# Safari77/rupphash

Measured on AMD Instinct MI355X. Metric: pdq_hashes_per_sec_512x512_rgb, higher is better.
Workload: dtype f32

## Files before the change

rupphash_amd/csrc/pdq_fused512.hip:

```cpp
#include "pdq_tail.hpp"
#include "rph_internal.h"

namespace {

typedef _Float16 h2 __attribute__((ext_vector_type(2)));
typedef _Float16 h8 __attribute__((ext_vector_type(8)));

template <int SW_, int CH_ = 3, bool PARK_ = true>
struct Geo {
    static constexpr int SW = SW_;
    static constexpr int CH = CH_;
    static constexpr int NSTRIP = 512 / SW;
    static constexpr int CL = SW / 8;
    static constexpr int NG = 64 / CL;
    static constexpr int NH = 64 / (NG * 8);
    static constexpr int NOCT = SW / 8;
    static constexpr int TILE_PITCH = SW * 2 + 16;
    static constexpr int TILE_BYTES = 64 * TILE_PITCH;
    static constexpr int OFF_TILE = 0;
    static constexpr int OFF_XCHG = NH == 2 ? 32 * TILE_PITCH : 0;
    static constexpr int OFF_STATE = TILE_BYTES;
    static constexpr int OFF_EDGE = OFF_STATE + 7168;
#ifndef RPH_PARK_CHAINS
#define RPH_PARK_CHAINS 1
#endif
    static constexpr bool PARK = RPH_PARK_CHAINS && PARK_ && SW == 64;
    static constexpr int OFF_PARK_C = OFF_EDGE + 1536;
    static constexpr int OFF_PARK_E = OFF_PARK_C + (PARK ? 9 * 64 * 4 : 0);
    static constexpr int LDS_BYTES = OFF_PARK_E + (PARK ? 9 * 6 * 4 : 0);
    static constexpr int WAVES_PER_SIMD = 2;
    static_assert(64 * 33 * 4 <= TILE_BYTES, "sample transpose buffer must fit in the dead V tile");
    static_assert((NG - 1) * 7 * CL * 16 <= (NH == 2 ? 32 : 64) * TILE_PITCH, "exchange area must fit");
    static_assert(rph::TAIL_LDS_FLOATS * 4 <= TILE_BYTES, "tail scratch must fit in the dead V tile");
};
constexpr int SAMP_PITCH = 33;

struct Px8 {
    uint32_t d[6];
};
struct __attribute__((packed, aligned(4))) U3 {
    uint32_t x, y, z;
};

struct __attribute__((packed, aligned(4))) U2 {
    uint32_t x, y;
};
template <int CH = 3>
__device__ __forceinline__ Px8 load_px8(const uint8_t *p)
{
    Px8 r;
    if (CH == 1) {
        const U2 a = *reinterpret_cast<const U2 *>(p);
        r.d[0] = a.x; r.d[1] = a.y; r.d[2] = r.d[3] = r.d[4] = r.d[5] = 0;
        return r;
    }
    const U3 a = *reinterpret_cast<const U3 *>(p);
    const U3 b = *reinterpret_cast<const U3 *>(p + 12);
    r.d[0] = a.x; r.d[1] = a.y; r.d[2] = a.z; r.d[3] = b.x; r.d[4] = b.y; r.d[5] = b.z;
    return r;
}

template <int P>
__device__ __forceinline__ float luma_px(const Px8 &v)
{
    constexpr int B = 3 * P;
    const float r = (float)((v.d[B >> 2] >> (8 * (B & 3))) & 0xFFu);
    const float g = (float)((v.d[(B + 1) >> 2] >> (8 * ((B + 1) & 3))) & 0xFFu);
    const float b = (float)((v.d[(B + 2) >> 2] >> (8 * ((B + 2) & 3))) & 0xFFu);
    const float num = __builtin_fmaf(299.0f, r, __builtin_fmaf(587.0f, g, __builtin_fmaf(114.0f, b, 500.0f)));
    return __builtin_truncf(num * 0.001f);
}

template <int CH = 3>
__device__ __forceinline__ void luma8(const Px8 &v, float (&l)[8])
{
    if (CH == 1) {
#pragma unroll
        for (int i = 0; i < 8; i++) l[i] = (float)((v.d[i >> 2] >> (8 * (i & 3))) & 0xFFu);
        return;
    }
    l[0] = luma_px<0>(v); l[1] = luma_px<1>(v); l[2] = luma_px<2>(v); l[3] = luma_px<3>(v);
    l[4] = luma_px<4>(v); l[5] = luma_px<5>(v); l[6] = luma_px<6>(v); l[7] = luma_px<7>(v);
}

constexpr uint32_t BIASED_ZERO = 0x64006400u;
struct Row8 {
    h2 q[4];
};
__device__ __forceinline__ h2 h2_bits(uint32_t u) { return __builtin_bit_cast(h2, u); }
__device__ __forceinline__ h2 byte_pair_lo(uint32_t d) { return h2_bits(__builtin_amdgcn_perm(0x64646464u, d, 0x04010400u)); }
__device__ __forceinline__ h2 byte_pair_hi(uint32_t d) { return h2_bits(__builtin_amdgcn_perm(0x64646464u, d, 0x04030402u)); }

__device__ __forceinline__ float dot2_from_zero(h2 a, h2 k, uint32_t after)
{
    float r;
    asm volatile("v_dot2_f32_f16 %0, %1, %2, 0" : "=v"(r) : "v"(__builtin_bit_cast(uint32_t, a)), "s"(__builtin_bit_cast(uint32_t, k)), "v"(after));
    return r;
}

struct Pairs12 {
    h2 P[12];
};
__device__ __forceinline__ Pairs12 byte_pairs(const Px8 &v)
{
    Pairs12 r;
#pragma unroll
    for (int i = 0; i < 6; i++) {
        r.P[2 * i] = byte_pair_lo(v.d[i]);
        r.P[2 * i + 1] = byte_pair_hi(v.d[i]);
    }
    return r;
}
__device__ __forceinline__ Row8 luma_row(const Pairs12 &pr, bool zero, uint32_t &order)
{
    const h2 *P = pr.P;
    const h2 k_rg = h2{(_Float16)299.0f, (_Float16)587.0f};
    const h2 k_b0 = h2{(_Float16)114.0f, (_Float16)0.0f};
    const h2 k_0r = h2{(_Float16)0.0f, (_Float16)299.0f};
    const h2 k_gb = h2{(_Float16)587.0f, (_Float16)114.0f};
    float vhalf;
    asm("v_mov_b32 %0, 0.5" : "=v"(vhalf));
    h2 packed[4];
#pragma unroll
    for (int pp = 0; pp < 4; pp++) {
        const float n0 = __builtin_amdgcn_fdot2(P[3 * pp], k_rg, dot2_from_zero(P[3 * pp + 1], k_b0, order), false);
        const float n1 = __builtin_amdgcn_fdot2(P[3 * pp + 1], k_0r, dot2_from_zero(P[3 * pp + 2], k_gb, order), false);
        const float y0 = __builtin_fmaf(n0, 0.001f, vhalf), y1 = __builtin_fmaf(n1, 0.001f, vhalf);
        packed[pp] = __builtin_bit_cast(h2, __builtin_amdgcn_cvt_pkrtz(y0, y1));
    }
    order = __builtin_bit_cast(uint32_t, packed[3]);
    Row8 r;
#pragma unroll
    for (int i = 0; i < 4; i++) {
        r.q[i] = packed[i];
        if (zero) r.q[i] = h2_bits(BIASED_ZERO);
    }
    return r;
}
__device__ __forceinline__ Row8 luma_row_gray(const Px8 &v, bool zero, uint32_t &order)
{
    Row8 r;
    r.q[0] = byte_pair_lo(v.d[0]);
    r.q[1] = byte_pair_hi(v.d[0]);
    r.q[2] = byte_pair_lo(v.d[1]);
    r.q[3] = byte_pair_hi(v.d[1]);
#pragma unroll
    for (int i = 0; i < 4; i++)
        if (zero) r.q[i] = h2_bits(BIASED_ZERO);
    order = __builtin_bit_cast(uint32_t, r.q[3]);
    return r;
}
template <int CH = 3>
__device__ __forceinline__ Row8 pack_row(const Px8 &v, bool zero, uint32_t &order)
{
    if (CH == 1) return luma_row_gray(v, zero, order);
    return luma_row(byte_pairs(v), zero, order);
}
__device__ __forceinline__ uint4 row_bits(const Row8 &r)
{
    uint4 u;
    u.x = __builtin_bit_cast(uint32_t, r.q[0]);
    u.y = __builtin_bit_cast(uint32_t, r.q[1]);
    u.z = __builtin_bit_cast(uint32_t, r.q[2]);
    u.w = __builtin_bit_cast(uint32_t, r.q[3]);
    return u;
}
__device__ __forceinline__ Row8 bits_row(const uint4 &u)
{
    Row8 r;
    r.q[0] = __builtin_bit_cast(h2, u.x);
    r.q[1] = __builtin_bit_cast(h2, u.y);
    r.q[2] = __builtin_bit_cast(h2, u.z);
    r.q[3] = __builtin_bit_cast(h2, u.w);
    return r;
}

__device__ __forceinline__ float div_small(float N, float d, float dinv)
{
    const float q0 = N * dinv;
    const float r = __builtin_fmaf(-q0, d, N);
    return __builtin_fmaf(r, dinv, q0);
}

__device__ __forceinline__ void wave_lds_fence() { asm volatile("" ::: "memory"); }

struct Wave {
    uint8_t *lds;
    const uint8_t *img;
    size_t row_stride;
    uint32_t rs32;
    int lane;
    float hs, sum, ring[8];
    uint4 pv;
    float row_d8, row_dinv8;
    float smp[32];
    float smp_last;
    float csum, cring[8];
    float ecs, ering[8];
    float bnew[8];
    rph::TailAcc tail;
    bool want_quality;
};

template <class G>
__device__ __forceinline__ int half_row(int b, int h, int g, int k) { return 64 * b + 4 + (G::NG * 8) * h + 8 * g + k; }

template <class G>
__device__ __forceinline__ void half_offsets(const Wave &w, int b, int s, int h, uint32_t &off0, uint32_t &off_max)
{
    const int c = w.lane & (G::CL - 1), g = w.lane / G::CL;
    const uint32_t col = (uint32_t)(G::SW * s + 8 * c) * (uint32_t)G::CH;
    off0 = (uint32_t)half_row<G>(b, h, g, 0) * w.rs32 + col;
    off_max = 511u * w.rs32 + col;
}
template <int CH>
__device__ __forceinline__ Px8 load_px8_at(const Wave &w, uint32_t off) { return load_px8<CH>(w.img + off); }

template <class G>
__device__ __forceinline__ void half_issue(const Wave &w, int b, int s, int h, Px8 (&pre)[8])
{
    uint32_t off, off_max;
    half_offsets<G>(w, b, s, h, off, off_max);
#pragma unroll
    for (int k = 0; k < 8; k++) {
        pre[k] = load_px8_at<G::CH>(w, off);
        off = off + w.rs32;
        off = off < off_max ? off : off_max;
    }
}

template <class G, bool LAST_BAND>
__device__ __forceinline__ void half_luma(const Wave &w, int b, int h, Px8 (&pre)[8], Row8 (&L)[8], bool has_next, int nb, int ns, int nh)
{
    const int g = w.lane / G::CL;
    uint32_t off, off_max;
    half_offsets<G>(w, nb, ns, nh, off, off_max);
    uint32_t order = 0;
#pragma unroll
    for (int k = 0; k < 8; k++) {
        if (G::CH == 1) {
            const Px8 cur = pre[k];
            if (has_next) pre[k] = load_px8_at<1>(w, off);
            off = off + w.rs32;
            off = off < off_max ? off : off_max;
            L[k] = luma_row_gray(cur, LAST_BAND && (half_row<G>(b, h, g, k) >= 512), order);
            continue;
        }
        const Pairs12 pr = byte_pairs(pre[k]);
        if (has_next) pre[k] = load_px8_at<3>(w, off);
        off = off + w.rs32;
        off = off < off_max ? off : off_max;
        L[k] = luma_row(pr, LAST_BAND && (half_row<G>(b, h, g, k) >= 512), order);
    }
}

template <class G>
__device__ __forceinline__ void half_build(Wave &w, int s, int h, const Row8 (&L)[8])
{
    const int c = w.lane & (G::CL - 1), g = w.lane / G::CL;
    uint8_t *tile = w.lds + G::OFF_TILE;
    uint8_t *xchg = w.lds + G::OFF_XCHG;
    uint8_t *state = w.lds + G::OFF_STATE + (G::SW * s + 8 * c) * 2;

    if (g < G::NG - 1) {
        uint8_t *x = xchg + ((g * 7) * G::CL + c) * 16;
#pragma unroll
        for (int k = 1; k < 8; k++) *reinterpret_cast<uint4 *>(x + (k - 1) * (G::CL * 16)) = row_bits(L[k]);
    }
    wave_lds_fence();
    Row8 hist[7];
    {
        const uint8_t *hp = (g == 0) ? state : xchg + (((g - 1) * 7) * G::CL + c) * 16;
        const int stride = (g == 0) ? 1024 : G::CL * 16;
#pragma unroll
        for (int j = 0; j < 7; j++) hist[j] = bits_row(*reinterpret_cast<const uint4 *>(hp + j * stride));
    }
    wave_lds_fence();
    if (g == G::NG - 1) {
#pragma unroll
        for (int k = 1; k < 8; k++) *reinterpret_cast<uint4 *>(state + (k - 1) * 1024) = row_bits(L[k]);
    }
    const int row0 = (G::NG * 8) * h + 8 * g;
    Row8 v;
#pragma unroll
    for (int i = 0; i < 4; i++) {
        const h2 two_bias = h2{(_Float16)2048.0f, (_Float16)2048.0f};
        h2 a = hist[0].q[i] + (hist[1].q[i] - two_bias);
        h2 bb = hist[2].q[i] + (hist[3].q[i] - two_bias);
        h2 cc = hist[4].q[i] + (hist[5].q[i] - two_bias);
        h2 dd = hist[6].q[i] + (L[0].q[i] - two_bias);
        v.q[i] = (a + bb) + (cc + dd);
    }
    *reinterpret_cast<uint4 *>(tile + (row0 + 0) * G::TILE_PITCH + 16 * c) = row_bits(v);
#pragma unroll
    for (int m = 1; m < 8; m++) {
#pragma unroll
        for (int i = 0; i < 4; i++) v.q[i] = (v.q[i] - hist[m - 1].q[i]) + L[m].q[i];
        *reinterpret_cast<uint4 *>(tile + (row0 + m) * G::TILE_PITCH + 16 * c) = row_bits(v);
    }
    wave_lds_fence();
}

__device__ __forceinline__ uint32_t h2_diff(uint32_t cur, uint32_t prev)
{
    return __builtin_bit_cast(uint32_t, __builtin_bit_cast(h2, cur) - __builtin_bit_cast(h2, prev));
}
template <int HI>
__device__ __forceinline__ float hs_step(float hs, uint32_t packed)
{
    float r;
    if (HI)
        asm("v_fma_mix_f32 %0, %1, 1.0, %2 op_sel:[1,0,0] op_sel_hi:[1,0,0]" : "=v"(r) : "v"(packed), "v"(hs));
    else
        asm("v_fma_mix_f32 %0, %1, 1.0, %2 op_sel:[0,0,0] op_sel_hi:[1,0,0]" : "=v"(r) : "v"(packed), "v"(hs));
    return r;
}
template <int HI>
__device__ __forceinline__ float hs_sub(float hs, uint32_t packed)
{
    float r;
    if (HI)
        asm("v_fma_mix_f32 %0, %1, -1.0, %2 op_sel:[1,0,0] op_sel_hi:[1,0,0]" : "=v"(r) : "v"(packed), "v"(hs));
    else
        asm("v_fma_mix_f32 %0, %1, -1.0, %2 op_sel:[0,0,0] op_sel_hi:[1,0,0]" : "=v"(r) : "v"(packed), "v"(hs));
    return r;
}

template <int E>
__device__ __forceinline__ void row_step(Wave &w, float in2)
{
    constexpr int slot = (E + 4) & 7;
    w.sum = w.sum + in2;
    w.sum = w.sum - w.ring[slot];
    w.ring[slot] = in2;
}

template <bool EDGE_ROWS>
__device__ __forceinline__ float pass1_value(const Wave &w, float hs)
{
    if (EDGE_ROWS) return div_small(hs, w.row_d8, w.row_dinv8);
    return hs;
}

template <class G, bool EDGE_ROWS, bool FIRST, bool LAST>
__device__ __forceinline__ void scan_strip(Wave &w)
{
    const int r = w.lane;
    const uint8_t *tp = w.lds + G::OFF_TILE + r * G::TILE_PITCH;
    const float *edge = reinterpret_cast<const float *>(w.lds + G::OFF_EDGE);
    float fresh[G::NOCT];
#pragma unroll
    for (int q = 0; q < G::NOCT; q++) {
        const uint4 cur = *reinterpret_cast<const uint4 *>(tp + 16 * q);
        const uint32_t dq[4] = {h2_diff(cur.x, w.pv.x), h2_diff(cur.y, w.pv.y), h2_diff(cur.z, w.pv.z), h2_diff(cur.w, w.pv.w)};
        const bool first_octet = FIRST && q == 0;
        float e0 = 0.f, e1 = 0.f, e2 = 0.f;
        if (first_octet) {
            e0 = edge[0 * 64 + r];
            e1 = edge[1 * 64 + r];
            e2 = edge[2 * 64 + r];
        }
#define RPH_STEP(E)                                                              \
    {                                                                            \
        w.hs = hs_step<(E) & 1>(w.hs, dq[(E) >> 1]);                             \
        float in2 = pass1_value<EDGE_ROWS>(w, w.hs);                             \
        if (first_octet && (E) == 4) in2 = e0;                                   \
        if (first_octet && (E) == 5) in2 = e1;                                   \
        if (first_octet && (E) == 6) in2 = e2;                                   \
        if (!(first_octet && (E) < 4)) row_step<E>(w, in2);  \
    }
        RPH_STEP(0) RPH_STEP(1) RPH_STEP(2) RPH_STEP(3) RPH_STEP(4)
        fresh[q] = w.sum * 0.125f;
        RPH_STEP(5) RPH_STEP(6) RPH_STEP(7)
#undef RPH_STEP
        w.pv = cur;
    }
    if (LAST) {
        const float e3 = edge[3 * 64 + r], e4 = edge[4 * 64 + r], e5 = edge[5 * 64 + r];
        w.hs = hs_sub<0>(w.hs, w.pv.x); row_step<0>(w, e3);
        w.hs = hs_sub<1>(w.hs, w.pv.x); row_step<1>(w, e4);
        w.hs = hs_sub<0>(w.hs, w.pv.y); row_step<2>(w, e5);
        w.hs = hs_sub<1>(w.hs, w.pv.y);
        {
            const float in511 = (EDGE_ROWS ? div_small(w.hs, w.row_d8, w.row_dinv8) : w.hs) * 2.0f;
            row_step<3>(w, in511);
        }
        w.sum = w.sum - w.ring[0];
        w.smp_last = w.sum / 7.0f;
    }
#pragma unroll
    for (int i = 0; i < 32 - G::NOCT; i++) w.smp[i] = w.smp[i + G::NOCT];
#pragma unroll
    for (int q = 0; q < G::NOCT; q++) w.smp[32 - G::NOCT + q] = fresh[q];
}

__device__ __forceinline__ void scan_reset(Wave &w, int b)
{
    w.hs = 0.f;
    w.sum = 0.f;
#pragma unroll
    for (int i = 0; i < 8; i++) w.ring[i] = 0.f;
    w.pv = make_uint4(0, 0, 0, 0);
    const int y = 64 * b + w.lane;
    const int lo = y - 3 < 0 ? 0 : y - 3, hi = y + 4 > 511 ? 511 : y + 4;
    const float d = (float)(hi - lo + 1);
    w.row_d8 = d * 0.125f;
    w.row_dinv8 = (1.0f / d) * 8.0f;
}

template <class G>
__device__ __forceinline__ void col_pass(Wave &w, int b, bool second_half)
{
    float *tb = reinterpret_cast<float *>(w.lds + G::OFF_TILE);
#pragma unroll
    for (int t = 0; t < 32; t++) tb[w.lane * SAMP_PITCH + t] = w.smp[t];
    tb[w.lane * SAMP_PITCH + 32] = w.smp_last;
    wave_lds_fence();
    const bool active = second_half ? (w.lane >= 31) : (w.lane < 31);
    if (active) {
        float *park = reinterpret_cast<float *>(w.lds + G::OFF_PARK_C) + w.lane;
        if (G::PARK) {
            w.csum = park[0];
#pragma unroll
            for (int e = 0; e < 8; e++) w.cring[e] = park[64 * (e + 1)];
        }
        const float *samp = tb + (second_half ? w.lane - 31 : w.lane + 1);
#pragma unroll
        for (int u = 0; u < 8; u++) {
            float in[8];
#pragma unroll
            for (int e = 0; e < 8; e++) in[e] = samp[(8 * u + e) * SAMP_PITCH];
#pragma unroll
            for (int e = 0; e < 8; e++) {
                w.csum = w.csum + in[e];
                w.csum = w.csum - w.cring[e];
                w.cring[e] = in[e];
                if (e == 0) w.bnew[u] = w.csum * (0.125f * 0.015625f);
            }
        }
        if (G::PARK) {
            park[0] = w.csum;
#pragma unroll
            for (int e = 0; e < 8; e++) park[64 * (e + 1)] = w.cring[e];
        }
    }
    wave_lds_fence();
}

template <int CH>
__device__ __forceinline__ void edge_rowvals(const Wave &w, int y, bool live, float (&rv)[6])
{
    const int yc = y > 511 ? 511 : y;
    const Px8 pl = load_px8<CH>(w.img + (size_t)yc * w.row_stride);
    const Px8 pr = load_px8<CH>(w.img + (size_t)yc * w.row_stride + 504 * CH);
    float l[8], r[8];
    luma8<CH>(pl, l);
    luma8<CH>(pr, r);
    const float r0 = (((l[0] + l[1]) + l[2]) + l[3]) + l[4];
    const float r1 = r0 + l[5];
    const float r2 = r1 + l[6];
    const float q510 = (((r[3] + r[4]) + r[5]) + r[6]) + r[7];
    const float q509 = q510 + r[2];
    const float q508 = q509 + r[1];
    rv[0] = div_small(r0 * 64.0f, 5.0f, 1.0f / 5.0f);
    rv[1] = div_small(r1 * 64.0f, 6.0f, 1.0f / 6.0f);
    rv[2] = div_small(r2 * 64.0f, 7.0f, 1.0f / 7.0f);
    rv[3] = div_small(q508 * 64.0f, 7.0f, 1.0f / 7.0f);
    rv[4] = div_small(q509 * 64.0f, 6.0f, 1.0f / 6.0f);
    rv[5] = div_small(q510 * 64.0f, 5.0f, 1.0f / 5.0f);
    if (!live) {
#pragma unroll
        for (int k = 0; k < 6; k++) rv[k] = 0.f;
    }
}

template <class G>
__device__ __forceinline__ void edge_prologue(Wave &w)
{
    float *edge = reinterpret_cast<float *>(w.lds + G::OFF_EDGE);
    float rv[6];
    edge_rowvals<G::CH>(w, w.lane & 3, true, rv);
    if (w.lane < 4) {
#pragma unroll
        for (int k = 0; k < 6; k++) edge[k * 64 + w.lane] = rv[k];
    }
    wave_lds_fence();
    w.ecs = 0.f;
#pragma unroll
    for (int i = 0; i < 8; i++) w.ering[i] = 0.f;
    if (w.lane < 6) {
#pragma unroll
        for (int t = 0; t < 4; t++) {
            const float v = edge[w.lane * 64 + t];
            w.ecs = w.ecs + v;
            w.ering[t] = v;
        }
        if (G::PARK) {
            float *park = reinterpret_cast<float *>(w.lds + G::OFF_PARK_E) + w.lane;
            park[0] = w.ecs;
#pragma unroll
            for (int i = 0; i < 8; i++) park[6 * (i + 1)] = w.ering[i];
        }
    }
    wave_lds_fence();
}

template <class G, int KIND>
__device__ __forceinline__ void edge_band(Wave &w, int b)
{
    float *edge = reinterpret_cast<float *>(w.lds + G::OFF_EDGE);
    {
        float rv[6];
        const int y = 64 * b + 4 + w.lane;
        edge_rowvals<G::CH>(w, y, y < 512, rv);
#pragma unroll
        for (int k = 0; k < 6; k++) edge[k * 64 + w.lane] = rv[k];
    }
    wave_lds_fence();
    if (w.lane < 6) {
        float *mine = edge + w.lane * 64;
        float *park = reinterpret_cast<float *>(w.lds + G::OFF_PARK_E) + w.lane;
        if (G::PARK) {
            w.ecs = park[0];
#pragma unroll
            for (int i = 0; i < 8; i++) w.ering[i] = park[6 * (i + 1)];
        }
#pragma unroll 1
        for (int u = 0; u < 8; u++) {
            float in[8], out[8];
#pragma unroll
            for (int e = 0; e < 8; e++) in[e] = mine[8 * u + e];
#pragma unroll
            for (int e = 0; e < 8; e++) {
                constexpr int dummy = 0;
                (void)dummy;
                const int slot = (e + 4) & 7;
                const bool add = !(KIND == 2 && u == 7 && e >= 4);
                if (add) w.ecs = w.ecs + in[e];
                w.ecs = w.ecs - w.ering[slot];
                w.ering[slot] = in[e];
                float o;
                if (KIND == 0 && u == 0 && e < 3)
                    o = w.ecs / (float)(5 + e);
                else if (KIND == 2 && u == 7 && e >= 4)
                    o = w.ecs / (float)(11 - e);
                else
                    o = w.ecs * 0.125f;
                out[e] = o;
            }
#pragma unroll
            for (int e = 0; e < 8; e++) mine[8 * u + e] = out[e];
        }
        if (G::PARK) {
            park[0] = w.ecs;
#pragma unroll
            for (int i = 0; i < 8; i++) park[6 * (i + 1)] = w.ering[i];
        }
    }
    wave_lds_fence();
}

template <class G>
__device__ __forceinline__ void store_samples(const Wave &w, float *band_samples, bool second_half)
{
    float *p = band_samples + (second_half ? 32 * 64 : 0) + w.lane;
    asm volatile("" : "+v"(p));
#pragma unroll
    for (int t = 0; t < 32; t++) p[t * 64] = w.smp[t];
    if (second_half) p[32 * 64] = w.smp_last;
}

template <class G, int KIND, bool LL = false>
__device__ __forceinline__ void do_band(Wave &w, int b, Px8 (&pre)[8], float *samples = nullptr)
{
    constexpr bool EDGE_ROWS = KIND != 1;
    if (!LL) edge_band<G, KIND>(w, b);
    scan_reset(w, b);
#pragma unroll 1
    for (int s = 0; s < G::NSTRIP; s++) {
#pragma unroll 1
        for (int h = 0; h < G::NH; h++) {
            Row8 L[8];
            int nb = b, ns = s, nh = h + 1;
            if (nh == G::NH) {
                nh = 0;
                ns = s + 1;
                if (ns == G::NSTRIP) {
                    ns = 0;
                    nb = b + 1;
                }
            }
            half_luma<G, KIND == 2>(w, b, h, pre, L, LL ? nb == b : nb < 8, nb, ns, nh);
            half_build<G>(w, s, h, L);
        }
        if (s == 0)
            scan_strip<G, EDGE_ROWS, true, false>(w);
        else if (s == G::NSTRIP - 1)
            scan_strip<G, EDGE_ROWS, false, true>(w);
        else
            scan_strip<G, EDGE_ROWS, false, false>(w);
        wave_lds_fence();
        if (LL) {
            if (s == G::NSTRIP / 2 - 1) store_samples<G>(w, samples, false);
            if (s == G::NSTRIP - 1) store_samples<G>(w, samples, true);
        } else {
            if (s == G::NSTRIP / 2 - 1) col_pass<G>(w, b, false);
            if (s == G::NSTRIP - 1) col_pass<G>(w, b, true);
        }
        wave_lds_fence();
    }
    if (LL) return;
#pragma unroll
    for (int u = 0; u < 8; u++)
        if (KIND != 0 || u > 0) rph::tail_row(w.tail, w.bnew[u], 8 * b + u - 1, w.lane, w.want_quality);
}

template <class G>
__global__ void __launch_bounds__(64, G::WAVES_PER_SIMD) pdq_fused512_kernel(const uint8_t *__restrict__ px, uint32_t n, size_t row_stride,
                                                          size_t image_stride, uint8_t *hash, float *quality, float *coeffs,
                                                          uint8_t *dihedral, uint8_t *valid)
{
    __shared__ __attribute__((aligned(16))) uint8_t lds[G::LDS_BYTES];
    const uint32_t img = blockIdx.x;
    Wave w;
    w.lds = lds;
    w.img = px + (size_t)img * image_stride;
    w.row_stride = row_stride;
    w.rs32 = (uint32_t)row_stride;
    w.lane = threadIdx.x;
    w.csum = 0.f;
    w.smp_last = 0.f;
#pragma unroll
    for (int i = 0; i < 32; i++) w.smp[i] = 0.f;
#pragma unroll
    for (int i = 0; i < 8; i++) w.cring[i] = 0.f;
    if (G::PARK) {
#pragma unroll
        for (int i = 0; i < 9; i++) reinterpret_cast<float *>(lds + G::OFF_PARK_C)[64 * i + w.lane] = 0.f;
    }
    rph::tail_init(w.tail);
    w.want_quality = quality != nullptr;
#pragma unroll
    for (int u = 0; u < 8; u++) w.bnew[u] = 0.f;

    {
        for (int j = 0; j < 3; j++)
            for (int t = w.lane; t < 64; t += 64) *reinterpret_cast<uint4 *>(lds + G::OFF_STATE + j * 1024 + t * 16) = make_uint4(BIASED_ZERO, BIASED_ZERO, BIASED_ZERO, BIASED_ZERO);
        uint32_t order = 0;
#pragma unroll 1
        for (int it = 0; it < 4; it++) {
            const int slot = it * 64 + w.lane;
            const int chunk = slot & 63, row = slot >> 6;
            const Px8 p = load_px8<G::CH>(w.img + (size_t)row * row_stride + (size_t)(8 * chunk) * G::CH);
            *reinterpret_cast<uint4 *>(lds + G::OFF_STATE + (3 + row) * 1024 + (8 * chunk) * 2) = row_bits(pack_row<G::CH>(p, false, order));
        }
    }
    edge_prologue<G>(w);

    Px8 pre[8];
    half_issue<G>(w, 0, 0, 0, pre);
    do_band<G, 0>(w, 0, pre);
#pragma unroll 1
    for (int b = 1; b < 7; b++) do_band<G, 1>(w, b, pre);
    do_band<G, 2>(w, 7, pre);

    if (G::PARK) {
        w.csum = reinterpret_cast<const float *>(lds + G::OFF_PARK_C)[w.lane];
        w.cring[0] = reinterpret_cast<const float *>(lds + G::OFF_PARK_C)[64 + w.lane];
    }
    w.csum = w.csum - w.cring[0];
    rph::tail_row(w.tail, (w.csum / 7.0f) * 0.015625f, 63, w.lane, w.want_quality);

    __syncthreads();
    rph::tail_finish(w.tail, reinterpret_cast<float *>(lds), w.lane, hash + (size_t)img * 32, quality ? quality + img : nullptr,
                  coeffs ? coeffs + (size_t)img * 256 : nullptr, dihedral ? dihedral + (size_t)img * 256 : nullptr);
    if (valid && w.lane == 0) valid[img] = 1;
}

constexpr int LL_SAMPLE_FLOATS = 8 * 65 * 64;
constexpr int LL_EDGE_PITCH = 520;

template <class G, int KIND>
__device__ __forceinline__ void ll_band(Wave &w, int b, float *samples)
{
    Px8 pre[8];
    half_issue<G>(w, b, 0, 0, pre);
    do_band<G, KIND, true>(w, b, pre, samples);
}

template <class G>
__global__ void __launch_bounds__(512, 2) pdq_fused512_ll_kernel(const uint8_t *__restrict__ px, uint32_t n, size_t row_stride, size_t image_stride,
                                                                 float *__restrict__ sample_scratch, uint8_t *hash, float *quality, float *coeffs,
                                                                 uint8_t *dihedral, uint8_t *valid)
{
    static_assert(G::NH == 1, "the low-latency kernel is built on the 64-px strip geometry");
    __shared__ __attribute__((aligned(16))) uint8_t lds[8 * G::LDS_BYTES + 6 * LL_EDGE_PITCH * 4];
    const uint32_t img = blockIdx.x;
    const int band = __builtin_amdgcn_readfirstlane(threadIdx.x >> 6);
    Wave w;
    w.lds = lds + band * G::LDS_BYTES;
    w.img = px + (size_t)img * image_stride;
    w.row_stride = row_stride;
    w.rs32 = (uint32_t)row_stride;
    w.lane = threadIdx.x & 63;
    w.smp_last = 0.f;
#pragma unroll
    for (int i = 0; i < 32; i++) w.smp[i] = 0.f;
    w.want_quality = quality != nullptr;
    float *edge_all = reinterpret_cast<float *>(lds + 8 * G::LDS_BYTES);
    float *samples = sample_scratch + (size_t)img * LL_SAMPLE_FLOATS;

    {
        float rv[6];
        edge_rowvals<G::CH>(w, 64 * band + w.lane, true, rv);
#pragma unroll
        for (int k = 0; k < 6; k++) edge_all[k * LL_EDGE_PITCH + 64 * band + w.lane] = rv[k];
        if (band == 7 && w.lane < 8) {
#pragma unroll
            for (int k = 0; k < 6; k++) edge_all[k * LL_EDGE_PITCH + 512 + w.lane] = 0.f;
        }
    }
    {
        uint32_t order = 0;
#pragma unroll 1
        for (int it = 0; it < 7; it++) {
            const int row = 64 * band - 3 + it;
            uint4 bits = make_uint4(BIASED_ZERO, BIASED_ZERO, BIASED_ZERO, BIASED_ZERO);
            if (row >= 0) bits = row_bits(pack_row<G::CH>(load_px8<G::CH>(w.img + (size_t)row * row_stride + (size_t)(8 * w.lane) * G::CH), false, order));
            *reinterpret_cast<uint4 *>(w.lds + G::OFF_STATE + it * 1024 + (8 * w.lane) * 2) = bits;
        }
    }
    __syncthreads();
    if (w.lane < 6) {
        const float *in = edge_all + w.lane * LL_EDGE_PITCH;
        float *mine = reinterpret_cast<float *>(w.lds + G::OFF_EDGE) + w.lane * 64;
        float ecs = 0.f, ering[8];
#pragma unroll
        for (int t = 0; t < 8; t++) ering[t] = 0.f;
#pragma unroll
        for (int t = 0; t < 4; t++) {
            ecs = ecs + in[t];
            ering[t] = in[t];
        }
#pragma unroll 1
        for (int bb = 0; bb < band; bb++)
#pragma unroll 1
            for (int u = 0; u < 8; u++) {
                float v[8];
#pragma unroll
                for (int e = 0; e < 8; e++) v[e] = in[64 * bb + 4 + 8 * u + e];
#pragma unroll
                for (int e = 0; e < 8; e++) {
                    ecs = ecs + v[e];
                    ecs = ecs - ering[(e + 4) & 7];
                    ering[(e + 4) & 7] = v[e];
                }
            }
#pragma unroll 1
        for (int u = 0; u < 8; u++) {
            float v[8], out[8];
#pragma unroll
            for (int e = 0; e < 8; e++) v[e] = in[64 * band + 4 + 8 * u + e];
#pragma unroll
            for (int e = 0; e < 8; e++) {
                const bool past_end = band == 7 && u == 7 && e >= 4;
                if (!past_end) ecs = ecs + v[e];
                ecs = ecs - ering[(e + 4) & 7];
                ering[(e + 4) & 7] = v[e];
                float o = ecs * 0.125f;
                if (band == 0 && u == 0 && e < 3) o = ecs / (float)(5 + e);
                if (past_end) o = ecs / (float)(11 - e);
                out[e] = o;
            }
#pragma unroll
            for (int e = 0; e < 8; e++) mine[8 * u + e] = out[e];
        }
    }
    wave_lds_fence();

    float *band_samples = samples + (size_t)band * (65 * 64);
    if (band == 0)
        ll_band<G, 0>(w, 0, band_samples);
    else if (band == 7)
        ll_band<G, 2>(w, 7, band_samples);
    else
        ll_band<G, 1>(w, band, band_samples);
    __syncthreads();
    if (band != 0) return;

    w.csum = 0.f;
#pragma unroll
    for (int i = 0; i < 8; i++) w.cring[i] = 0.f;
    rph::tail_init(w.tail);
    const float *col = samples + (size_t)(w.lane + 1) * 64;
#pragma unroll 1
    for (int bb = 0; bb < 8; bb++) {
        const float *cb = col + (size_t)bb * (65 * 64);
#pragma unroll 1
        for (int u = 0; u < 8; u++) {
            const float4 lo = *reinterpret_cast<const float4 *>(cb + 8 * u), hi = *reinterpret_cast<const float4 *>(cb + 8 * u + 4);
            const float in[8] = {lo.x, lo.y, lo.z, lo.w, hi.x, hi.y, hi.z, hi.w};
            float bnew = 0.f;
#pragma unroll
            for (int e = 0; e < 8; e++) {
                w.csum = w.csum + in[e];
                w.csum = w.csum - w.cring[e];
                w.cring[e] = in[e];
                if (e == 0) bnew = w.csum * (0.125f * 0.015625f);
            }
            if (bb != 0 || u != 0) rph::tail_row(w.tail, bnew, 8 * bb + u - 1, w.lane, w.want_quality);
        }
    }
    w.csum = w.csum - w.cring[0];
    rph::tail_row(w.tail, (w.csum / 7.0f) * 0.015625f, 63, w.lane, w.want_quality);
    wave_lds_fence();
    rph::tail_finish(w.tail, reinterpret_cast<float *>(w.lds), w.lane, hash + (size_t)img * 32, quality ? quality + img : nullptr,
                     coeffs ? coeffs + (size_t)img * 256 : nullptr, dihedral ? dihedral + (size_t)img * 256 : nullptr);
    if (valid && w.lane == 0) valid[img] = 1;
}

}

int rph_launch_pdq_fused512_ll(rph_ctx *ctx, const uint8_t *d_px, uint32_t n, size_t row_stride, size_t image_stride, uint8_t *d_hash,
                               float *d_quality, float *d_coeffs, uint8_t *d_dihedral, uint8_t *d_valid, hipStream_t stream)
{
    if (n == 0) return RPH_OK;
    const uint32_t chunk = n < 256 ? n : 256;
    const size_t need = (size_t)chunk * LL_SAMPLE_FLOATS * sizeof(float);
    if (ctx->ll_scratch.size() > 256 && ctx->ll_scratch.find(stream) == ctx->ll_scratch.end()) {
        RPH_HIP_CHECK(hipDeviceSynchronize());
        ctx->ll_scratch.clear();
    }
    DevBuf &sc = ctx->ll_scratch[stream];
    RPH_TRY(sc.reserve(need, stream));
    for (uint32_t first = 0; first < n; first += chunk) {
        const uint32_t m = (n - first) < chunk ? (n - first) : chunk;
        hipLaunchKernelGGL((pdq_fused512_ll_kernel<Geo<64, 3, false>>), dim3(m), dim3(512), 0, stream, d_px + (size_t)first * image_stride, m, row_stride, image_stride,
                           sc.as<float>(), d_hash + (size_t)first * 32, d_quality ? d_quality + first : nullptr, d_coeffs ? d_coeffs + (size_t)first * 256 : nullptr,
                           d_dihedral ? d_dihedral + (size_t)first * 256 : nullptr, d_valid ? d_valid + first : nullptr);
        RPH_HIP_CHECK(hipGetLastError());
    }
    return RPH_OK;
}

int rph_launch_pdq_fused512(rph_ctx *ctx, const uint8_t *d_px, uint32_t n, size_t row_stride, size_t image_stride,
                            uint8_t *d_hash, float *d_quality, float *d_coeffs, uint8_t *d_dihedral, uint8_t *d_valid,
                            hipStream_t stream, uint32_t channels)
{
    if (n == 0) return RPH_OK;
    if (channels == 1) {
        hipLaunchKernelGGL((pdq_fused512_kernel<Geo<64, 1>>), dim3(n), dim3(64), 0, stream, d_px, n, row_stride, image_stride, d_hash, d_quality, d_coeffs, d_dihedral,
                           d_valid);
        RPH_HIP_CHECK(hipGetLastError());
        return RPH_OK;
    }
    if (ctx->pdq_kernel == 3 || ((ctx->pdq_kernel == 4 || ctx->pdq_kernel == 6) && n < 768))
        return rph_launch_pdq_fused512_ll(ctx, d_px, n, row_stride, image_stride, d_hash, d_quality, d_coeffs, d_dihedral, d_valid, stream);
    if (ctx->pdq_kernel == 2)
        hipLaunchKernelGGL(pdq_fused512_kernel<Geo<128>>, dim3(n), dim3(64), 0, stream, d_px, n, row_stride, image_stride, d_hash,
                           d_quality, d_coeffs, d_dihedral, d_valid);
    else
        hipLaunchKernelGGL(pdq_fused512_kernel<Geo<64>>, dim3(n), dim3(64), 0, stream, d_px, n, row_stride, image_stride, d_hash,
                           d_quality, d_coeffs, d_dihedral, d_valid);
    RPH_HIP_CHECK(hipGetLastError());
    return RPH_OK;
}
```

Baseline: 6.787 million.

## Prefetch next band's edge rows during column pass and hoist head loads

Splits the edge-row computation into separate load issue and compute steps, so the global loads for the next band's edge rows are issued inside the final column pass of the current band. The first four image rows, the band-0 edge rows and the first strip prefetch are all issued at kernel entry. The edge prologue now reads its luma from the already packed fp16 rows in LDS instead of reloading from global memory. The aim is to hide global-load latency behind LDS and ALU work, at the cost of more live registers (extra Px8 buffers) and possibly lower occupancy.

Result: faster. 6.934 million, median of 6 (+2.2%).

```diff
diff --git a/rupphash_amd/csrc/pdq_fused512.hip b/rupphash_amd/csrc/pdq_fused512.hip
--- a/rupphash_amd/csrc/pdq_fused512.hip
+++ b/rupphash_amd/csrc/pdq_fused512.hip
@@ -29,6 +29,7 @@
     static constexpr int OFF_PARK_E = OFF_PARK_C + (PARK ? 9 * 64 * 4 : 0);
     static constexpr int LDS_BYTES = OFF_PARK_E + (PARK ? 9 * 6 * 4 : 0);
     static constexpr int WAVES_PER_SIMD = 2;
+    static constexpr bool AHEAD = SW == 64;
     static_assert(64 * 33 * 4 <= TILE_BYTES, "sample transpose buffer must fit in the dead V tile");
     static_assert((NG - 1) * 7 * CL * 16 <= (NH == 2 ? 32 : 64) * TILE_PITCH, "exchange area must fit");
     static_assert(rph::TAIL_LDS_FLOATS * 4 <= TILE_BYTES, "tail scratch must fit in the dead V tile");
@@ -408,13 +409,14 @@
     w.row_dinv8 = (1.0f / d) * 8.0f;
 }
 
-template <class G>
-__device__ __forceinline__ void col_pass(Wave &w, int b, bool second_half)
+template <class G, bool NEXT_EDGE = false>
+__device__ __forceinline__ void col_pass(Wave &w, int b, bool second_half, Px8 (*epx)[2] = nullptr)
 {
     float *tb = reinterpret_cast<float *>(w.lds + G::OFF_TILE);
 #pragma unroll
     for (int t = 0; t < 32; t++) tb[w.lane * SAMP_PITCH + t] = w.smp[t];
     tb[w.lane * SAMP_PITCH + 32] = w.smp_last;
+    if (NEXT_EDGE) edge_band_issue<G>(w, b + 1, *epx);
     wave_lds_fence();
     const bool active = second_half ? (w.lane >= 31) : (w.lane < 31);
     if (active) {
@@ -448,14 +450,14 @@
 }
 
 template <int CH>
-__device__ __forceinline__ void edge_rowvals(const Wave &w, int y, bool live, float (&rv)[6])
+__device__ __forceinline__ void edge_issue(const Wave &w, int y, Px8 (&e)[2])
 {
     const int yc = y > 511 ? 511 : y;
-    const Px8 pl = load_px8<CH>(w.img + (size_t)yc * w.row_stride);
-    const Px8 pr = load_px8<CH>(w.img + (size_t)yc * w.row_stride + 504 * CH);
-    float l[8], r[8];
-    luma8<CH>(pl, l);
-    luma8<CH>(pr, r);
+    e[0] = load_px8<CH>(w.img + (size_t)yc * w.row_stride);
+    e[1] = load_px8<CH>(w.img + (size_t)yc * w.row_stride + 504 * CH);
+}
+__device__ __forceinline__ void edge_values(const float (&l)[8], const float (&r)[8], bool live, float (&rv)[6])
+{
     const float r0 = (((l[0] + l[1]) + l[2]) + l[3]) + l[4];
     const float r1 = r0 + l[5];
     const float r2 = r1 + l[6];
@@ -473,13 +475,38 @@
         for (int k = 0; k < 6; k++) rv[k] = 0.f;
     }
 }
+template <int CH>
+__device__ __forceinline__ void edge_compute(const Px8 (&e)[2], bool live, float (&rv)[6])
+{
+    float l[8], r[8];
+    luma8<CH>(e[0], l);
+    luma8<CH>(e[1], r);
+    edge_values(l, r, live, rv);
+}
+template <int CH>
+__device__ __forceinline__ void edge_rowvals(const Wave &w, int y, bool live, float (&rv)[6])
+{
+    Px8 e[2];
+    edge_issue<CH>(w, y, e);
+    edge_compute<CH>(e, live, rv);
+}
 
 template <class G>
 __device__ __forceinline__ void edge_prologue(Wave &w)
 {
     float *edge = reinterpret_cast<float *>(w.lds + G::OFF_EDGE);
     float rv[6];
-    edge_rowvals<G::CH>(w, w.lane & 3, true, rv);
+    {
+        const uint8_t *row = w.lds + G::OFF_STATE + (3 + (w.lane & 3)) * 1024;
+        const h8 hl = *reinterpret_cast<const h8 *>(row), hr = *reinterpret_cast<const h8 *>(row + 504 * 2);
+        float l[8], r[8];
+#pragma unroll
+        for (int i = 0; i < 8; i++) {
+            l[i] = (float)hl[i] - 1024.0f;
+            r[i] = (float)hr[i] - 1024.0f;
+        }
+        edge_values(l, r, true, rv);
+    }
     if (w.lane < 4) {
 #pragma unroll
         for (int k = 0; k < 6; k++) edge[k * 64 + w.lane] = rv[k];
@@ -505,14 +532,17 @@
     wave_lds_fence();
 }
 
+template <class G>
+__device__ __forceinline__ void edge_band_issue(const Wave &w, int b, Px8 (&epx)[2]) { edge_issue<G::CH>(w, 64 * b + 4 + w.lane, epx); }
+
 template <class G, int KIND>
-__device__ __forceinline__ void edge_band(Wave &w, int b)
+__device__ __forceinline__ void edge_band(Wave &w, int b, const Px8 (&epx)[2])
 {
     float *edge = reinterpret_cast<float *>(w.lds + G::OFF_EDGE);
     {
         float rv[6];
         const int y = 64 * b + 4 + w.lane;
-        edge_rowvals<G::CH>(w, y, y < 512, rv);
+        edge_compute<G::CH>(epx, y < 512, rv);
 #pragma unroll
         for (int k = 0; k < 6; k++) edge[k * 64 + w.lane] = rv[k];
     }
@@ -571,10 +601,13 @@
 }
 
 template <class G, int KIND, bool LL = false>
-__device__ __forceinline__ void do_band(Wave &w, int b, Px8 (&pre)[8], float *samples = nullptr)
+__device__ __forceinline__ void do_band(Wave &w, int b, Px8 (&pre)[8], float *samples, Px8 (&epx)[2])
 {
     constexpr bool EDGE_ROWS = KIND != 1;
-    if (!LL) edge_band<G, KIND>(w, b);
+    if (!LL) {
+        if (!G::AHEAD) edge_band_issue<G>(w, b, epx);
+        edge_band<G, KIND>(w, b, epx);
+    }
     scan_reset(w, b);
 #pragma unroll 1
     for (int s = 0; s < G::NSTRIP; s++) {
@@ -605,11 +638,15 @@
             if (s == G::NSTRIP - 1) store_samples<G>(w, samples, true);
         } else {
             if (s == G::NSTRIP / 2 - 1) col_pass<G>(w, b, false);
-            if (s == G::NSTRIP - 1) col_pass<G>(w, b, true);
+            if (!G::AHEAD && s == G::NSTRIP - 1) col_pass<G>(w, b, true);
         }
         wave_lds_fence();
     }
     if (LL) return;
+    if (G::AHEAD) {
+        col_pass<G, KIND != 2>(w, b, true, &epx);
+        wave_lds_fence();
+    }
 #pragma unroll
     for (int u = 0; u < 8; u++)
         if (KIND != 0 || u > 0) rph::tail_row(w.tail, w.bnew[u], 8 * b + u - 1, w.lane, w.want_quality);
@@ -628,6 +665,14 @@
     w.row_stride = row_stride;
     w.rs32 = (uint32_t)row_stride;
     w.lane = threadIdx.x;
+    Px8 head[4], epx[2], pre[8];
+    if (G::AHEAD) {
+#pragma unroll
+        for (int row = 0; row < 4; row++) head[row] = load_px8<G::CH>(w.img + (size_t)row * row_stride + (size_t)(8 * w.lane) * G::CH);
+        edge_band_issue<G>(w, 0, epx);
+    }
+    half_issue<G>(w, 0, 0, 0, pre);
+    wave_lds_fence();
     w.csum = 0.f;
     w.smp_last = 0.f;
 #pragma unroll
@@ -647,22 +692,27 @@
         for (int j = 0; j < 3; j++)
             for (int t = w.lane; t < 64; t += 64) *reinterpret_cast<uint4 *>(lds + G::OFF_STATE + j * 1024 + t * 16) = make_uint4(BIASED_ZERO, BIASED_ZERO, BIASED_ZERO, BIASED_ZERO);
         uint32_t order = 0;
-#pragma unroll 1
-        for (int it = 0; it < 4; it++) {
-            const int slot = it * 64 + w.lane;
-            const int chunk = slot & 63, row = slot >> 6;
-            const Px8 p = load_px8<G::CH>(w.img + (size_t)row * row_stride + (size_t)(8 * chunk) * G::CH);
-            *reinterpret_cast<uint4 *>(lds + G::OFF_STATE + (3 + row) * 1024 + (8 * chunk) * 2) = row_bits(pack_row<G::CH>(p, false, order));
-        }
-    }
+        if (G::AHEAD) {
+#pragma unroll
+            for (int row = 0; row < 4; row++)
+                *reinterpret_cast<uint4 *>(lds + G::OFF_STATE + (3 + row) * 1024 + (8 * w.lane) * 2) = row_bits(pack_row<G::CH>(head[row], false, order));
+        } else {
+#pragma unroll 1
+            for (int it = 0; it < 4; it++) {
+                const int slot = it * 64 + w.lane;
+                const int chunk = slot & 63, row = slot >> 6;
+                const Px8 p = load_px8<G::CH>(w.img + (size_t)row * row_stride + (size_t)(8 * chunk) * G::CH);
+                *reinterpret_cast<uint4 *>(lds + G::OFF_STATE + (3 + row) * 1024 + (8 * chunk) * 2) = row_bits(pack_row<G::CH>(p, false, order));
+            }
+        }
+    }
+    wave_lds_fence();
     edge_prologue<G>(w);
 
-    Px8 pre[8];
-    half_issue<G>(w, 0, 0, 0, pre);
-    do_band<G, 0>(w, 0, pre);
-#pragma unroll 1
-    for (int b = 1; b < 7; b++) do_band<G, 1>(w, b, pre);
-    do_band<G, 2>(w, 7, pre);
+    do_band<G, 0>(w, 0, pre, nullptr, epx);
+#pragma unroll 1
+    for (int b = 1; b < 7; b++) do_band<G, 1>(w, b, pre, nullptr, epx);
+    do_band<G, 2>(w, 7, pre, nullptr, epx);
 
     if (G::PARK) {
         w.csum = reinterpret_cast<const float *>(lds + G::OFF_PARK_C)[w.lane];
@@ -685,7 +735,8 @@
 {
     Px8 pre[8];
     half_issue<G>(w, b, 0, 0, pre);
-    do_band<G, KIND, true>(w, b, pre, samples);
+    Px8 none[2];
+    do_band<G, KIND, true>(w, b, pre, samples, none);
 }
 
 template <class G>
```
